# wildsonbbl/gnnepcsaft

Hardware: AMD Instinct MI355X
Metric: molecular graphs/sec (fwd+bwd) (higher is better)
Workload: dtype f32; 1 GPU; BASELINE configs[1]: PNA hidden=128 L=6 towers=1 pre=2 post=4, 4096 graphs/GPU (81920 atoms, 163840 directed bonds), fwd+loss+bwd incl. CSR packing; graphs_per_gpu=4096, parallelism=dp1, hip_graph=False, launch=auto, grad_allreduce_bytes=0, grad_exchange=none (1 rank)

## Files before the change

gnnepcsaft_amd/_lib.py:

```python
from __future__ import annotations

import ctypes as C
from pathlib import Path
from typing import Dict, Optional

import torch

_LIB_PATH = Path(__file__).resolve().parent / "libgnnepcsaft_hip.so"

ABI_VERSION = 7
GNX_OK, GNX_E_INVALID, GNX_E_HIP, GNX_E_RANGE, GNX_E_WORKSPACE = 0, -1, -2, -3, -4
OPT_GEMM_SPLIT, OPT_WGRAD_WGS, OPT_EMBED_BWD_MFMA, OPT_STD_BWD_CENTERED, OPT_GEMM_PIPE, OPT_WGRAD_PIPE, OPT_GEMM_AS, \
    OPT_GEMM_WS_FAST, OPT_GEMM_TILE_ROWS, OPT_GEMM_MID = range(10)
GEMM_RELU, GEMM_ACCUMULATE, GEMM_B_TRANS, GEMM_SPLIT_ONLY, GEMM_PRESPLIT = 1, 2, 4, 8, 16
GEMM_KERNEL_NAMES = ("none", "k_gemm<vec>", "k_gemm<generic>", "k_gemm_ws", "k_gemm_ws3", "k_gemm_ws3<fast,8>",
                     "k_gemm_ws3<fast,4>", "k_gemm3", "k_gemm3p<96>", "k_gemm3p<128>", "k_gemm_as3", "k_gemm_mid",
                     "k_gemm_small_batched")
POOL_ADD, POOL_MEAN, POOL_MAX = 0, 1, 2
K_NONE, K_PNA_AGG_FWD, K_PNA_AGG_BWD, K_GEMM_WS, K_GEMM_WGRAD, K_GINE_AGG_FWD, K_GINE_AGG_BWD, K_EDGE_COMBINE_FWD, \
    K_EDGE_COMBINE_BWD, K_BN_FWD, K_BN_BWD, K_GEMM_TILED, K_GEMM_SMALL, K_GEMM_WGRAD_BATCHED, K_KEY_SEGMENT_SUM, \
    K_EMBED, K_PNA_EDGE_FWD, K_PNA_EDGE_BWD, K_ATTN_FWD, K_ATTN_BWD, K_PCSAFT_RHO, K_PCSAFT_VP, \
    K_PCSAFT_MIX_STATE, K_PCSAFT_MIX_RHO, K_PCSAFT_MIX_LNPHI_STATE, K_PCSAFT_MIX_LNPHI = range(26)
K_COUNT = 26
KERNEL_GROUPS = {K_PNA_AGG_FWD: "pna_aggregate_fwd", K_PNA_AGG_BWD: "pna_aggregate_bwd", K_GEMM_WS: "gemm_weights_stationary",
                 K_GEMM_WGRAD: "weight_gradient", K_GINE_AGG_FWD: "gine_aggregate_fwd", K_GINE_AGG_BWD: "gine_aggregate_bwd",
                 K_EDGE_COMBINE_FWD: "edge_combine_fwd", K_EDGE_COMBINE_BWD: "edge_combine_bwd", K_BN_FWD: "batchnorm_fwd",
                 K_BN_BWD: "batchnorm_bwd", K_GEMM_TILED: "gemm_tiled", K_GEMM_SMALL: "gemm_small",
                 K_GEMM_WGRAD_BATCHED: "weight_gradient_batched", K_KEY_SEGMENT_SUM: "key_segment_sum", K_EMBED: "embedding",
                 K_PNA_EDGE_FWD: "pna_edge_fused_fwd", K_PNA_EDGE_BWD: "pna_edge_fused_bwd",
                 K_ATTN_FWD: "transformer_attn_fwd", K_ATTN_BWD: "transformer_attn_bwd",
                 K_PCSAFT_RHO: "pcsaft_density", K_PCSAFT_VP: "pcsaft_vapor_pressure",
                 K_PCSAFT_MIX_STATE: "pcsaft_mix_state", K_PCSAFT_MIX_RHO: "pcsaft_mix_density",
                 K_PCSAFT_MIX_LNPHI_STATE: "pcsaft_mix_lnphi_state", K_PCSAFT_MIX_LNPHI: "pcsaft_mix_lnphi"}


class GnxError(RuntimeError):
    def __init__(self, status: int, msg: str):
        super().__init__(f"gnx status {status}: {msg}")
        self.status = status


class GemmSeg(C.Structure):
    _fields_ = [("a", C.c_void_p), ("lda", C.c_int64), ("rowscale", C.c_void_p), ("b", C.c_void_p),
                ("ldb", C.c_int64), ("k", C.c_int32), ("_pad", C.c_int32)]


class GemmPlanInfo(C.Structure):
    _fields_ = [("kernel", C.c_int32), ("tile_rows", C.c_int32), ("grid_x", C.c_uint32), ("grid_y", C.c_uint32),
                ("block", C.c_uint32), ("runs_split", C.c_int32), ("image_bytes", C.c_size_t)]


class WgradProb(C.Structure):
    _fields_ = [("dC", C.c_void_p), ("lddc", C.c_int64), ("A", C.c_void_p), ("lda", C.c_int64),
                ("rowscale", C.c_void_p), ("dW", C.c_void_p), ("lddw", C.c_int64), ("dbias", C.c_void_p),
                ("M", C.c_int64), ("N", C.c_int32), ("K", C.c_int32)]


_vp, _i32, _i64, _f32, _sz = C.c_void_p, C.c_int32, C.c_int64, C.c_float, C.c_size_t

PNA_MAX_LAYERS, PNA_MAX_TOWERS = 8, 8
PNA_BWD_DEFER_SMALL, PNA_BWD_LAST_OF_PASS = 1, 2


class PnaFwdArgs(C.Structure):
    _fields_ = [("N", _i64), ("E", _i64), ("T", _i32), ("F", _i32), ("pre_layers", _i32), ("post_layers", _i32),
                ("D", _i32), ("merged", _i32),
                ("rowptr", _vp), ("src", _vp), ("dst", _vp), ("code", _vp), ("dperm", _vp), ("tiles", _vp), ("ntiles", _vp),
                ("max_tiles", _i64), ("x", _vp), ("Te", _vp), ("weff", _vp * PNA_MAX_TOWERS), ("Wm", _vp), ("bm", _vp),
                ("params", C.POINTER(_vp)), ("P", _vp), ("Q", _vp), ("A", _vp), ("hs", _vp * PNA_MAX_LAYERS),
                ("zs", _vp * PNA_MAX_LAYERS), ("ws", _vp), ("ws_bytes", _sz), ("out", _vp), ("etile_info", _vp),
                ("etile_w", _i32), ("tile_rows", _i32)]


class PnaBwdArgs(C.Structure):
    _fields_ = [("N", _i64), ("E", _i64), ("T", _i32), ("F", _i32), ("pre_layers", _i32), ("post_layers", _i32),
                ("R", _i32), ("D", _i32), ("avg_deg_log", _f32), ("merged", _i32), ("acc_first", _i32),
                ("use_side_streams", _i32), ("n_h", _i32), ("n_z", _i32),
                ("rowptr", _vp), ("colptr", _vp), ("cpos", _vp), ("code", _vp), ("code_pos", _vp), ("dperm", _vp),
                ("tiles", _vp), ("ntiles", _vp), ("chunks", _vp), ("nchunks", _vp),
                ("max_tiles", _i64), ("max_chunks", _i64),
                ("x", _vp), ("BE", _vp), ("EE", _vp), ("A", _vp),
                ("hs", _vp * PNA_MAX_LAYERS), ("zs", _vp * PNA_MAX_LAYERS), ("weff", _vp * PNA_MAX_TOWERS), ("Wm", _vp),
# ... 57 lines not shown
                             C.POINTER(C.c_double), C.POINTER(C.c_double)]),
    "gnx_prof_end": (_i32, [_vp]),
    "gnx_pack_csr_workspace_bytes": (_sz, [_i64, _i64]),
    "gnx_pack_csr": (_i32, [_vp, _vp, _i64, _i64, _vp, _vp, _vp, _vp, _vp, _vp, _vp, _sz]),
    "gnx_feature_code": (_i32, [_vp, _vp, _i64, _i32, C.POINTER(_i32), _vp, _vp, _vp, _sz]),
    "gnx_graph_ptr": (_i32, [_vp, _vp, _i64, _i64, _vp, _vp, _sz]),
    "gnx_degree_scalers": (_i32, [_vp, _vp, _i64, _f32, _vp, _vp]),
    "gnx_embed_sum_fwd": (_i32, [_vp, _vp, _i64, _i32, C.POINTER(_i32), _vp, _i32, _vp]),
    "gnx_table_scatter_workspace_bytes": (_sz, [_i64, _i32, _i32]),
    "gnx_embed_sum_bwd": (_i32, [_vp, _vp, _i64, _i32, C.POINTER(_i32), _i32, _vp, _i32, _vp, _vp, _sz]),
    "gnx_check_range": (_i32, [_vp]),
    "gnx_collate_ptr": (_i32, [_vp, _vp, _vp, _i64, _vp, _i64, _vp, _vp]),
    "gnx_collate_gather": (_i32, [_vp, _vp, _vp, _i64, _vp, _vp, _vp, _i64, _vp, _i64, _vp, _vp, _i64, _i64, _vp, _vp,
                                  _vp, _vp]),
    "gnx_collate_rows": (_i32, [_vp, _vp, _i64, _vp, _i64, _i32, _i32, _vp]),
    "gnx_gemm_workspace_bytes": (_sz, [_vp, _i32, C.POINTER(GemmSeg), C.POINTER(_i64), _i32, _i64, _i32, _vp, _i32,
                                       _i32]),
    "gnx_gemm": (_i32, [_vp, _i32, C.POINTER(GemmSeg), _i64, _i32, _vp, _vp, _i64, _vp, _i64, _i32, _vp, _sz]),
    "gnx_gemm_wgrad": (_i32, [_vp, _vp, _i64, _vp, _i64, _vp, _i64, _i32, _i32, _vp, _i64, _vp]),
    "gnx_gemm_wgrad_batched": (_i32, [_vp, _i32, C.POINTER(WgradProb)]),
    "gnx_degree_max": (_i32, [_vp, _vp, _i64, C.POINTER(_i32)]),
    "gnx_degree_classes_workspace_bytes": (_sz, [_i64, _i32]),
    "gnx_degree_classes": (_i32, [_vp, _vp, _i64, _i32, _vp, _vp, _vp, _sz]),
    "gnx_class_tiles": (_i32, [_vp, _vp, _i32, _i32, _vp, _vp]),
    "gnx_gemm_grouped": (_i32, [_vp, _i32, C.POINTER(GemmSeg), C.POINTER(_i64), _i32, _i64, _i32, _vp, _vp, _i64, _vp,
                                _i64, _i32, _vp, _vp, _vp, _i64, _vp, _sz]),
    "gnx_gemm_tile_rows": (_i32, [_vp, _i64, _i32]),
    "gnx_gemm_grouped_rows": (_i32, [_vp, _i32, C.POINTER(GemmSeg), C.POINTER(_i64), _i32, _i64, _i32, _vp, _vp, _i64, _vp,
                                     _i64, _i32, _vp, _vp, _vp, _i64, _vp, _sz, _i32]),
    "gnx_gemm_plan": (_i32, [_vp, _i32, C.POINTER(GemmSeg), C.POINTER(_i64), _i32, _i64, _i32, _vp, _vp, _i64, _vp, _i64, _i32,
                             _vp, _vp, _vp, _i64, _vp, _sz, _i32, C.POINTER(GemmPlanInfo)]),
    "gnx_gemm_wgrad_grouped": (_i32, [_vp, _vp, _i64, _vp, _i64, _i64, _i32, _i32, _vp, _i64, _i64, _vp, _vp, _vp,
                                      _i64]),
    "gnx_pna_weff": (_i32, [_vp, _vp, _i64, _i32, _i32, _f32, _vp]),
    "gnx_pna_weff_bwd": (_i32, [_vp, _vp, _i32, _i32, _f32, _vp, _i64]),
    "gnx_group_by_small_key": (_i32, [_vp, _vp, _i64, _i32, _vp, _vp, _vp, _sz]),
    "gnx_key_segment_sum": (_i32, [_vp, _vp, _vp, _vp, _i64, _i32, _vp]),
    "gnx_edge_combine_fwd": (_i32, [_vp, _vp, _vp, _vp, _vp, _vp, _vp, _i64, _i32, _i32, _vp]),
    "gnx_edge_combine_bwd": (_i32, [_vp, _vp, _vp, _vp, _vp, _vp, _i64, _i64, _i32, _i32, _vp, _vp, _vp, _vp, _sz]),
    "gnx_pna_aggregate_fwd": (_i32, [_vp, _vp, _vp, _i64, _i64, _i32, _i32, _vp]),
    "gnx_pna_aggregate_bwd": (_i32, [_vp, _vp, _vp, _vp, _vp, _i64, _i64, _i32, _i32, _vp]),
    "gnx_edge_tiles_count": (_i32, [_i64, _i32]),
    "gnx_edge_tiles": (_i32, [_vp, _vp, _i64, _i64, _i32, _vp]),
    "gnx_pack_batch_workspace_bytes": (_sz, [_i64, _i64, _i32, _i32]),
    "gnx_pack_batch": (_i32, [_vp, C.POINTER(PackBatchArgs)]),
    "gnx_pack_batch_scan_chunk": (_i64, []),
    "gnx_pack_batch_scan_bound": (_i64, []),
    "gnx_pna_edge_fwd": (_i32, [_vp, _vp, _vp, _vp, _vp, _vp, _vp, _vp, _vp, _i32, _i64, _i64, _i32, _i32, C.POINTER(_vp),
                                C.POINTER(_vp), _vp, _vp, _vp]),
    "gnx_pna_edge_bwd": (_i32, [_vp, _vp, _vp, _vp, _vp, _vp, _i32, _i64, _i64, _i32, _i32, _i32, C.POINTER(_vp), _vp, _vp,
                                _vp]),
    "gnx_gine_aggregate_fwd": (_i32, [_vp, _vp, _vp, _vp, _vp, _vp, _i64, _i64, _i32, _f32, _vp]),
    "gnx_gine_aggregate_bwd": (_i32, [_vp, _vp, _vp, _vp, _vp, _vp, _vp, _vp, _vp, _vp, _i64, _i64, _i32, _i32, _f32,
                                      _vp, _vp]),
    "gnx_gine_dle": (_i32, [_vp, _vp, _vp, _vp, _vp, _vp, _vp, _vp, _i64, _i32, _i32, _vp]),
    "gnx_transformer_attn_fwd": (_i32, [_vp, _vp, _vp, _vp, _vp, _vp, _i64, _i64, _i32, _i32, _f32, C.c_uint64,
                                        C.c_uint64, _vp, _vp, _vp]),
    "gnx_transformer_attn_bwd": (_i32, [_vp, _vp, _vp, _vp, _vp, _vp, _vp, _vp, _vp, _vp, _vp, _vp, _i64, _i64, _i32,
                                        _i32, _i32, _f32, C.c_uint64, C.c_uint64, _vp, _vp, _vp]),
    "gnx_transformer_attn_dle": (_i32, [_vp, _vp, _vp, _vp, _vp, _vp, _vp, _i64, _i32, _i32, _i32, _vp]),
    "gnx_pcsaft_density": (_i32, [_vp, _vp, _i64, _vp, _vp, _vp, _i64, _vp, _vp]),
    "gnx_pcsaft_vapor_pressure": (_i32, [_vp, _vp, _i64, _vp, _vp, _i64, _vp, _vp, _vp, _vp]),
    "gnx_pcsaft_mix_state": (_i32, [_vp, _vp, _i64, _vp, _vp, _vp, _i64, _i32, _vp, _vp, _vp, _vp, _i64, _vp, _vp, _vp,
                                    _vp]),
    "gnx_pcsaft_mix_density": (_i32, [_vp, _vp, _i64, _vp, _vp, _vp, _i64, _i32, _vp, _vp, _vp, _vp, _i64, _vp, _vp]),
    "gnx_pcsaft_mix_lnphi_state": (_i32, [_vp, _vp, _i64, _vp, _vp, _vp, _i64, _i32, _vp, _vp, _vp, _vp, _i64, _vp, _vp,
# ... 117 lines not shown
```

gnnepcsaft_amd/csrc/gnx_wgrad.hip:

```cpp
#include "gnx_split.hpp"

struct wgrad_args {
  const float* X;
  int64_t ldx;
  const float* Y;
  int64_t ldy;
  const float* rs;
  int64_t M;
  int N, K;
  float* dW;
  int64_t lddw;
  float* dbias;
  int64_t rows_per_block;
  int vec_x, vec_y;
  const int* row_index;
  const int* chunk_info;
  const int* nchunks;
  int64_t dw_cls_stride;
  const float* zero;
};

template <bool VEC, bool GROUPED>
__device__ __forceinline__ void wgrad_body(const wgrad_args& g, const int bx, const int by, const int bz, float* Xs,
                                           float* Ys) {
  const int tid = threadIdx.x;
  const int lane = tid & 63;
  const int wave = tid >> 6;
  const int wm = wave >> 1, wn = wave & 1;
  const int li = lane & 31, lh = lane >> 5;
  const int n0 = by * BN;
  const int c0 = bz * BN;
  if (n0 >= g.N || c0 >= g.K) return;
  int64_t r_begin = (int64_t)bx * g.rows_per_block;
// ... 285 lines not shown
      for (int mi = 0; mi < 2; ++mi)
#pragma unroll
        for (int ni = 0; ni < 2; ++ni) mfma_3x3(acc[mi][ni], a[mi], b[ni]);
    }
  }

#pragma unroll
  for (int mi = 0; mi < 2; ++mi)
#pragma unroll
    for (int ni = 0; ni < 2; ++ni) {
      int gc = c0 + wn * 64 + ni * 32 + li;
      if (gc >= g.K) continue;
#pragma unroll
      for (int r = 0; r < 16; ++r) {
        int gr = n0 + wm * 64 + mi * 32 + (r & 3) + 8 * (r >> 2) + 4 * lh;
        if (gr >= g.N) continue;
        atomicAdd(dW + (int64_t)gr * g.lddw + gc, acc[mi][ni][r]);
      }
    }
  if (g.dbias != nullptr && bz == 0 && x_ok) atomicAdd(g.dbias + n0 + col, bsum);
}

template <bool GROUPED>
__global__ void __launch_bounds__(256, 2) k_gemm_wgrad3(wgrad_args g) {
  __shared__ __attribute__((aligned(16))) unsigned char A3[G3_OP];
  __shared__ __attribute__((aligned(16))) unsigned char B3[G3_OP];
  __shared__ __attribute__((aligned(16))) unsigned offs[128];
  wgrad3_body<GROUPED>(g, blockIdx.x, blockIdx.y, blockIdx.z, A3, B3, offs);
}

#define WG3P_LDS (4 * G3_OP)
#define WG3P_NST 4

__device__ __forceinline__ void wgrad3p_body(const wgrad_args& g, const int bx, const int by, const int bz,
                                             unsigned char* lds) {
  const int tid = threadIdx.x;
  const int lane = tid & 63;
  const int wave = tid >> 6;
  const int n0 = by * BN;
  const int c0 = bz * BN;
  if (n0 >= g.N || c0 >= g.K) return;
  int64_t r_begin = (int64_t)bx * g.rows_per_block;
  int64_t r_end = r_begin + g.rows_per_block;
  if (r_end > g.M) r_end = g.M;
  float* const dW = g.dW;
  if (r_begin >= r_end) return;
  const int64_t nsteps = (r_end - r_begin + BK - 1) / BK;

  if (wave < 4) {
    const int wm = wave >> 1, wn = wave & 1;
    const int li = lane & 31, lh = lane >> 5;
    f32x16 acc[2][2];
#pragma unroll
    for (int i = 0; i < 2; ++i)
#pragma unroll
      for (int j = 0; j < 2; ++j)
#pragma unroll
        for (int r = 0; r < 16; ++r) acc[i][j][r] = 0.f;
    __syncthreads();
    for (int64_t j = 0; j < nsteps; ++j) {
      const unsigned char* const A3 = lds + (j & 1) * 2 * G3_OP;
      const unsigned char* const B3 = A3 + G3_OP;
#pragma unroll
      for (int sl = 0; sl < 2; ++sl) {
        bf16x8 a[2][3], b[2][3];
#pragma unroll
// ... 73 lines not shown
  load_step(std::integral_constant<int, 0>{}, row_of(0));
  load_step(std::integral_constant<int, 1>{}, row_of(1));
  load_step(std::integral_constant<int, 2>{}, row_of(2));
  load_step(std::integral_constant<int, 3>{}, row_of(3));
  store_step(std::integral_constant<int, 0>{}, lds);
  load_step(std::integral_constant<int, 0>{}, row_of(4));
  __syncthreads();

  auto iteration = [&](auto KC, int64_t j) {
    constexpr int K = decltype(KC)::value;
    constexpr int P = (K + 1) % WG3P_NST;
    store_step(std::integral_constant<int, P>{}, lds + ((K + 1) & 1) * 2 * G3_OP);
    load_step(std::integral_constant<int, P>{}, row_of(j + 1 + WG3P_NST));
    __syncthreads();
  };
  for (int64_t j = 0; j < nsteps; j += 4) {
    iteration(std::integral_constant<int, 0>{}, j);
    if (j + 1 >= nsteps) break;
    iteration(std::integral_constant<int, 1>{}, j + 1);
    if (j + 2 >= nsteps) break;
    iteration(std::integral_constant<int, 2>{}, j + 2);
    if (j + 3 >= nsteps) break;
    iteration(std::integral_constant<int, 3>{}, j + 3);
  }
  if (g.dbias != nullptr && bz == 0 && role == 0 && col_ok) {
#pragma unroll
    for (int q = 0; q < 4; ++q) atomicAdd(g.dbias + n0 + c4 + q, bsum[q]);
  }
}

__global__ void __launch_bounds__(512, 1) k_gemm_wgrad3p(wgrad_args g) {
  extern __shared__ __attribute__((aligned(16))) unsigned char lds_w[];
  wgrad3p_body(g, blockIdx.x, blockIdx.y, blockIdx.z, lds_w);
}

#define WGRAD_MAX_BATCH 8
struct wgrad_batch_args {
  wgrad_args p[WGRAD_MAX_BATCH];
  int nprob;
  int wg_off[WGRAD_MAX_BATCH + 1];
  int tiles_k[WGRAD_MAX_BATCH];
  int tiles[WGRAD_MAX_BATCH];
};

__device__ __forceinline__ void wgrad_batch_locate(const wgrad_batch_args& b, int w, int& prob, int& chunk, int& by,
                                                   int& bz) {
  prob = 0;
#pragma unroll
  for (int i = 1; i < WGRAD_MAX_BATCH; ++i) prob += (i < b.nprob && w >= b.wg_off[i]) ? 1 : 0;
  int off = b.wg_off[0], tiles = b.tiles[0], tk = b.tiles_k[0];
#pragma unroll
  for (int i = 1; i < WGRAD_MAX_BATCH; ++i)
    if (i == prob) {
      off = b.wg_off[i];
      tiles = b.tiles[i];
      tk = b.tiles_k[i];
    }
  const int local = w - off;
  chunk = local / tiles;
  const int t = local - chunk * tiles;
  by = t / tk;
  bz = t - by * tk;
}

__global__ void __launch_bounds__(256, 2) k_gemm_wgrad_batched(wgrad_batch_args b) {
  __shared__ __attribute__((aligned(16))) float Xs[BK * LDN];
// ... 20 lines not shown
}

__global__ void __launch_bounds__(512, 1) k_gemm_wgrad3p_batched(wgrad_batch_args b) {
  extern __shared__ __attribute__((aligned(16))) unsigned char lds_wb[];
  int prob, chunk, by, bz;
  wgrad_batch_locate(b, blockIdx.x, prob, chunk, by, bz);
  wgrad_args g = b.p[0];
#pragma unroll
  for (int i = 1; i < WGRAD_MAX_BATCH; ++i)
    if (i == prob) g = b.p[i];
  wgrad3p_body(g, chunk, by, bz, lds_wb);
}

static wgrad_args wgrad_args_of(const gnx_handle* h, const gnx_wgrad_prob& q) {
  wgrad_args g = {};
  g.X = q.dC;
  g.ldx = q.lddc;
  g.Y = q.A;
  g.ldy = q.lda;
  g.rs = q.rowscale;
  g.M = q.M;
  g.N = q.N;
  g.K = q.K;
  g.dW = q.dW;
  g.lddw = q.lddw;
  g.dbias = q.dbias;
  g.vec_x = aligned16(q.dC) && (q.lddc % 4 == 0);
  g.vec_y = aligned16(q.A) && (q.lda % 4 == 0);
  g.zero = h->d_zero;
  return g;
}

static bool wgrad_split_enabled(const gnx_handle* h, int64_t M, bool any_rowscale) {
  if (any_rowscale || M < 4096) return false;
  return h->opt[GNX_OPT_GEMM_SPLIT] != 0;
}

static int32_t wgrad_launch(gnx_handle* h, const float* dC, int64_t lddc, const float* A, int64_t lda,
                            const float* rowscale, int64_t M, int32_t N, int32_t K, float* dW, int64_t lddw,
                            float* dbias, const int32_t* row_index, const int32_t* chunk_info, const int32_t* nchunks,
                            int64_t max_chunks, int64_t dw_cls_stride) {
  GNX_CHECK_ARG(h && dC && A && dW, "gnx_gemm_wgrad: NULL argument");
  GNX_CHECK_ARG(M >= 0 && N > 0 && K > 0 && lddc >= N && lda >= K && lddw >= K, "gnx_gemm_wgrad: bad shape");
  if (M == 0) return GNX_OK;
  wgrad_args g = wgrad_args_of(h, gnx_wgrad_prob{dC, lddc, A, lda, rowscale, dW, lddw, dbias, M, N, K});
  int64_t tiles = gnx_cdiv(N, BN) * gnx_cdiv(K, BN);
  const int64_t target_wgs = h->opt[GNX_OPT_WGRAD_WGS] > 0 ? h->opt[GNX_OPT_WGRAD_WGS] : (h->num_cus > 0 ? h->num_cus : 256);
  int64_t chunks = gnx_cdiv(target_wgs, tiles);
  int64_t rows = gnx_cdiv(gnx_cdiv(M, chunks), BK) * BK;
  if (rows < 128) rows = 128;
  g.rows_per_block = rows;
  g.row_index = row_index;
  g.chunk_info = chunk_info;
  g.nchunks = nchunks;
  g.dw_cls_stride = dw_cls_stride;
  dim3 grid((unsigned)(chunk_info ? max_chunks : gnx_cdiv(M, rows)), (unsigned)gnx_cdiv(N, BN), (unsigned)gnx_cdiv(K, BN));
  const bool vec = g.vec_x && g.vec_y && (N % 4 == 0) && (K % 4 == 0);
  const bool offs32 = (uint64_t)M * (uint64_t)lddc < (1ull << 32) && (uint64_t)M * (uint64_t)lda < (1ull << 32);
  const bool wsplit = wgrad_split_enabled(h, M, rowscale != nullptr) && (!chunk_info || offs32);
  const double wfl = 2.0 * (double)M * N * K;
  gnx_prof_scope prof(h, GNX_K_GEMM_WGRAD, 4.0 * M * ((double)N + K) + 4.0 * N * K, wfl, wsplit ? 6.0 * wfl : 0.0);
  if (wsplit && vec && !chunk_info && rows >= 512 && h->opt[GNX_OPT_WGRAD_PIPE] != 0) {
    GNX_HIP(gnx_raise_lds_limit<&k_gemm_wgrad3p>((int)WG3P_LDS));
    hipLaunchKernelGGL(k_gemm_wgrad3p, grid, dim3(512), WG3P_LDS, h->stream, g);
  } else if (wsplit) {
    if (chunk_info)
      hipLaunchKernelGGL((k_gemm_wgrad3<true>), grid, dim3(256), 0, h->stream, g);
    else
      hipLaunchKernelGGL((k_gemm_wgrad3<false>), grid, dim3(256), 0, h->stream, g);
  } else if (chunk_info) {
    if (vec)
      hipLaunchKernelGGL((k_gemm_wgrad<true, true>), grid, dim3(256), 0, h->stream, g);
    else
      hipLaunchKernelGGL((k_gemm_wgrad<false, true>), grid, dim3(256), 0, h->stream, g);
  } else {
    if (vec)
      hipLaunchKernelGGL((k_gemm_wgrad<true, false>), grid, dim3(256), 0, h->stream, g);
    else
      hipLaunchKernelGGL((k_gemm_wgrad<false, false>), grid, dim3(256), 0, h->stream, g);
  }
  GNX_LAUNCH_CHECK();
  return GNX_OK;
}

extern "C" int32_t gnx_gemm_wgrad(gnx_handle* h, const float* dC, int64_t lddc, const float* A, int64_t lda,
                                  const float* rowscale, int64_t M, int32_t N, int32_t K, float* dW, int64_t lddw,
                                  float* dbias) {
  return wgrad_launch(h, dC, lddc, A, lda, rowscale, M, N, K, dW, lddw, dbias, nullptr, nullptr, nullptr, 0, 0);
}

extern "C" int32_t gnx_gemm_wgrad_grouped(gnx_handle* h, const float* dC, int64_t lddc, const float* A, int64_t lda,
                                          int64_t M, int32_t N, int32_t K, float* dW_cls, int64_t lddw,
                                          int64_t dw_cls_stride, const int32_t* row_index, const int32_t* chunk_info,
                                          const int32_t* nchunks, int64_t max_chunks) {
  GNX_CHECK_ARG(row_index && chunk_info && nchunks && max_chunks > 0, "gnx_gemm_wgrad_grouped: NULL argument");
  return wgrad_launch(h, dC, lddc, A, lda, nullptr, M, N, K, dW_cls, lddw, nullptr, row_index, chunk_info, nchunks,
                      max_chunks, dw_cls_stride);
}

extern "C" int32_t gnx_gemm_wgrad_batched(gnx_handle* h, int32_t nprob, const gnx_wgrad_prob* probs) {
  GNX_CHECK_ARG(h && probs && nprob >= 1 && nprob <= WGRAD_MAX_BATCH, "gnx_gemm_wgrad_batched: nprob must be in [1,%d]",
                WGRAD_MAX_BATCH);
  wgrad_batch_args b;
  int64_t maxM = 0;
  int maxN = 0, maxK = 0;
  for (int i = 0; i < nprob; ++i) {
    const gnx_wgrad_prob& q = probs[i];
    GNX_CHECK_ARG(q.dC && q.A && q.dW && q.M >= 0 && q.N > 0 && q.K > 0 && q.lddc >= q.N && q.lda >= q.K && q.lddw >= q.K,
                  "gnx_gemm_wgrad_batched: problem %d: bad argument", i);
    b.p[i] = wgrad_args_of(h, q);
    GNX_CHECK_ARG(b.p[i].vec_x && b.p[i].vec_y && (q.N % 4 == 0) && (q.K % 4 == 0),
                  "gnx_gemm_wgrad_batched: problem %d is not 16-byte aligned / multiple-of-4 shaped", i);
    if (q.M > maxM) maxM = q.M;
    if (q.N > maxN) maxN = q.N;
    if (q.K > maxK) maxK = q.K;
  }
  for (int i = nprob; i < WGRAD_MAX_BATCH; ++i) b.p[i] = b.p[0];
  if (maxM == 0) return GNX_OK;
  double total_cost = 0.0;
  for (int i = 0; i < nprob; ++i)
    total_cost += (double)b.p[i].M * (double)(gnx_cdiv(b.p[i].N, BN) * gnx_cdiv(b.p[i].K, BN));
  int off = 0;
  for (int i = 0; i < WGRAD_MAX_BATCH; ++i) {
    b.wg_off[i] = off;
    b.tiles[i] = 1;
    b.tiles_k[i] = 1;
    if (i >= nprob) continue;
    const int tn = (int)gnx_cdiv(b.p[i].N, BN), tk = (int)gnx_cdiv(b.p[i].K, BN);
    const int64_t M = b.p[i].M > 0 ? b.p[i].M : 1;
    const double cus_d = (double)(h->num_cus > 0 ? h->num_cus : 256);
// ... 37 lines not shown
```

gnnepcsaft_amd/ops.py:

```python
from __future__ import annotations

import ctypes as C
import threading
from typing import List, Optional, Sequence, Tuple

import torch

from . import _lib
from ._lib import GemmSeg, check, handle

_I32 = C.c_int32


def _f32(t: torch.Tensor, name: str) -> torch.Tensor:
    if t.dtype != torch.float32:
        raise _lib.GnxError(_lib.GNX_E_INVALID, f"{name}: expected float32, got {t.dtype}")
    return t


def _mat(t: torch.Tensor, name: str) -> Tuple[int, int]:
    if t.dtype is not torch.float32:
        raise _lib.GnxError(_lib.GNX_E_INVALID, f"{name}: expected float32, got {t.dtype}")
    shape, strides = t.shape, t.stride()
    if len(shape) != 2 or (shape[1] > 1 and strides[1] != 1):
# ... 447 lines not shown
                 mask: Optional[torch.Tensor] = None, relu: bool = False, b_trans: bool = True,
                 forward_tiles: bool = False) -> torch.Tensor:
    if out.size(0) == 0:
        return out
    a, _ws = _gemm_args(segs, out, dc, bias, mask, relu, False, b_trans, forward_tiles)
    lib = _lib.load()
    check(lib.gnx_gemm_grouped_rows(*a) if forward_tiles else lib.gnx_gemm_grouped(*a[:19]))
    return out


def gemm_plan(segs, out: torch.Tensor, *, bias: Optional[torch.Tensor] = None, mask: Optional[torch.Tensor] = None,
              relu: bool = False, accumulate: bool = False, b_trans: bool = True, dc: Optional[DegreeClasses] = None,
              forward_tiles: bool = False) -> Tuple[str, "_lib.GemmPlanInfo"]:
    a, _ws = _gemm_args(segs, out, dc, bias, mask, relu, accumulate, b_trans, forward_tiles)
    info = _lib.GemmPlanInfo()
    check(_lib.load().gnx_gemm_plan(*a, C.byref(info)))
    return _lib.GEMM_KERNEL_NAMES[info.kernel], info


def gemm_wgrad_grouped(dC: torch.Tensor, A: torch.Tensor, dW_cls: torch.Tensor, dc: DegreeClasses) -> None:
    M, N = dC.shape
    if M == 0:
        return
    xp, ldx = _mat(dC, "dC")
    ap, lda = _mat(A, "A")
    K = A.size(1)
    if dW_cls.shape != (dc.D, N, K) or not dW_cls.is_contiguous():
        raise _lib.GnxError(_lib.GNX_E_INVALID, f"dW_cls must be contiguous [{dc.D},{N},{K}], got {tuple(dW_cls.shape)}")
    check(_lib.load().gnx_gemm_wgrad_grouped(handle(dC.device), xp, ldx, ap, lda, M, N, K, dW_cls.data_ptr(), K, N * K,
                                             dc.dperm.data_ptr(), dc.chunks.data_ptr(), dc.nchunks.data_ptr(),
                                             dc.max_chunks))


def pna_weff(W: torch.Tensor, F: int, D: int, avg_deg_log: float) -> torch.Tensor:
    wp, ldw = _mat(W, "W")
    out = torch.empty(D, F, 4 * F, dtype=torch.float32, device=W.device)
    check(_lib.load().gnx_pna_weff(handle(W.device), wp, ldw, F, D, float(avg_deg_log), out.data_ptr()))
    return out


def pna_weff_bwd(dWeff: torch.Tensor, F: int, D: int, avg_deg_log: float, dW: torch.Tensor) -> None:
    wp, ldw = _mat(dW, "dW")
    check(_lib.load().gnx_pna_weff_bwd(handle(dW.device), dWeff.data_ptr(), F, D, float(avg_deg_log), wp, ldw))


_SIDE_ENABLED = False
_SIDE_PENDING = set()
_SIDE_KEEP: dict = {}


def set_wgrad_side_stream(enabled: bool) -> None:
    global _SIDE_ENABLED
    _SIDE_ENABLED = bool(enabled)


_JOIN_QUEUED = False


_SIDE_USED: dict = {}


def _join(idx: int, which: Optional[int] = None) -> None:
    dev = torch.device("cuda", idx)
    used = _SIDE_USED.get(idx, set())
    for w in sorted(used if which is None else (used & {which})):
        check(_lib.load().gnx_side_join_n(handle(dev), w))
# ... 721 lines not shown
```

include/gnx.h:

```cpp
#ifndef GNX_H_
#define GNX_H_

#include <stddef.h>
#include <stdint.h>

#ifdef __cplusplus
extern "C" {
#endif

#define GNX_ABI_VERSION 7

enum {
  GNX_OK = 0,
  GNX_E_INVALID = -1,
  GNX_E_HIP = -2,
  GNX_E_RANGE = -3,
  GNX_E_WORKSPACE = -4
};

typedef struct gnx_handle gnx_handle;

int32_t gnx_create(gnx_handle** out, int32_t device);
int32_t gnx_destroy(gnx_handle* h);
int32_t gnx_set_stream(gnx_handle* h, void* hip_stream);
// ... 147 lines not shown
                              size_t ws_bytes, int32_t tile_rows);
enum {
  GNX_GEMM_KERNEL_NONE = 0,
  GNX_GEMM_KERNEL_TILED_VEC = 1,
  GNX_GEMM_KERNEL_TILED_GENERIC = 2,
  GNX_GEMM_KERNEL_WS = 3,
  GNX_GEMM_KERNEL_WS3 = 4,
  GNX_GEMM_KERNEL_WS3_FAST8 = 5,
  GNX_GEMM_KERNEL_WS3_FAST4 = 6,
  GNX_GEMM_KERNEL_GEMM3 = 7,
  GNX_GEMM_KERNEL_GEMM3P_96 = 8,
  GNX_GEMM_KERNEL_GEMM3P_128 = 9,
  GNX_GEMM_KERNEL_AS3 = 10,
  GNX_GEMM_KERNEL_MID = 11,
  GNX_GEMM_KERNEL_SMALL = 12,
  GNX_GEMM_KERNEL_COUNT = 13
};
typedef struct {
  int32_t kernel;
  int32_t tile_rows;
  uint32_t grid_x, grid_y, block;
  int32_t runs_split;
  size_t image_bytes;
} gnx_gemm_plan_info;
int32_t gnx_gemm_plan(gnx_handle* h, int32_t nseg, const gnx_gemm_seg* segs, const int64_t* cls_strides,
                      int32_t num_classes, int64_t M, int32_t N, const float* bias, const float* mask, int64_t ldmask,
                      float* C, int64_t ldc, int32_t flags, const int32_t* row_index, const int32_t* tile_info,
                      const int32_t* ntiles, int64_t max_tiles, void* ws, size_t ws_bytes, int32_t tile_rows,
                      gnx_gemm_plan_info* out);
int32_t gnx_gemm_wgrad_grouped(gnx_handle* h, const float* dC, int64_t lddc, const float* A, int64_t lda, int64_t M,
                               int32_t N, int32_t K, float* dW_cls, int64_t lddw, int64_t dw_cls_stride,
                               const int32_t* row_index, const int32_t* chunk_info, const int32_t* nchunks,
                               int64_t max_chunks);
int32_t gnx_pna_weff(gnx_handle* h, const float* W, int64_t ldw, int32_t F, int32_t D, float avg_deg_log, float* Weff);
int32_t gnx_pna_weff_bwd(gnx_handle* h, const float* dWeff, int32_t F, int32_t D, float avg_deg_log, float* dW,
                         int64_t lddw);
int32_t gnx_pna_weff_batched(gnx_handle* h, int32_t n, const float* const* W, int64_t ldw, int32_t F, int32_t D,
                             const float* avg_deg_log, float* const* Weff);
int32_t gnx_pna_weff_bwd_batched(gnx_handle* h, int32_t n, const float* const* dWeff, int32_t F, int32_t D,
                                 const float* avg_deg_log, float* const* dW, int64_t lddw);

int32_t gnx_edge_combine_fwd(gnx_handle* h, const float* P, const float* Q, const float* Te, const int32_t* src,
                             const int32_t* dst, const int32_t* code, int64_t E, int32_t H, int32_t relu, float* h1);
int32_t gnx_edge_combine_bwd(gnx_handle* h, const float* g, const int32_t* rowptr, const int32_t* colptr,
                             const int32_t* cpos, const int32_t* code, int64_t N, int64_t E, int32_t H, int32_t R,
                             float* dP, float* dQ, float* dTe, void* ws, size_t ws_bytes);

int32_t gnx_group_by_small_key(gnx_handle* h, const int32_t* keys, int64_t E, int32_t R, int32_t* pos, int32_t* ptr,
                               void* ws, size_t ws_bytes);
int32_t gnx_key_segment_sum(gnx_handle* h, const float* g, const int32_t* pos, const int32_t* key, int64_t E, int32_t H,
                            float* dtable);

int32_t gnx_pna_aggregate_fwd(gnx_handle* h, const float* m, const int32_t* rowptr, int64_t N, int64_t E, int32_t T,
                              int32_t F, float* A);
int32_t gnx_pna_aggregate_bwd(gnx_handle* h, const float* dA, const float* m, const float* A, const int32_t* rowptr,
                              int64_t N, int64_t E, int32_t T, int32_t F, float* dm);

int32_t gnx_edge_tiles_count(int64_t E, int32_t tile_w);
int32_t gnx_edge_tiles(gnx_handle* h, const int32_t* rowptr, int64_t N, int64_t E, int32_t tile_w, int32_t* tile_info);

#define GNX_PACK_MAX_AVG 4
#define GNX_PACK_CLASSES 1u
#define GNX_PACK_CODE_INDEX 2u
#define GNX_PACK_EDGE_TILES 4u
#define GNX_PACK_TILED_SCAN 256u
typedef struct {
// ... 262 lines not shown
```

Baseline: 639,600 graphs/s.

## Add warp-specialized pipelined split-bf16 kernel for grouped weight gradients

```diff
diff --git a/gnnepcsaft_amd/_lib.py b/gnnepcsaft_amd/_lib.py
--- a/gnnepcsaft_amd/_lib.py
+++ b/gnnepcsaft_amd/_lib.py
@@ -16,6 +16,8 @@
 GEMM_KERNEL_NAMES = ("none", "k_gemm<vec>", "k_gemm<generic>", "k_gemm_ws", "k_gemm_ws3", "k_gemm_ws3<fast,8>",
                      "k_gemm_ws3<fast,4>", "k_gemm3", "k_gemm3p<96>", "k_gemm3p<128>", "k_gemm_as3", "k_gemm_mid",
                      "k_gemm_small_batched")
+WGRAD_KERNEL_NAMES = ("none", "k_gemm_wgrad<true,true>", "k_gemm_wgrad<false,true>", "k_gemm_wgrad3<true>",
+                      "k_gemm_wgrad3p_grouped")
 POOL_ADD, POOL_MEAN, POOL_MAX = 0, 1, 2
 K_NONE, K_PNA_AGG_FWD, K_PNA_AGG_BWD, K_GEMM_WS, K_GEMM_WGRAD, K_GINE_AGG_FWD, K_GINE_AGG_BWD, K_EDGE_COMBINE_FWD, \
     K_EDGE_COMBINE_BWD, K_BN_FWD, K_BN_BWD, K_GEMM_TILED, K_GEMM_SMALL, K_GEMM_WGRAD_BATCHED, K_KEY_SEGMENT_SUM, \
@@ -48,6 +50,11 @@
 class GemmPlanInfo(C.Structure):
     _fields_ = [("kernel", C.c_int32), ("tile_rows", C.c_int32), ("grid_x", C.c_uint32), ("grid_y", C.c_uint32),
                 ("block", C.c_uint32), ("runs_split", C.c_int32), ("image_bytes", C.c_size_t)]
+
+
+class WgradGroupedPlanInfo(C.Structure):
+    _fields_ = [("kernel", C.c_int32), ("ranges", C.c_int32), ("chunks_per_range", C.c_int32), ("grid_x", C.c_uint32),
+                ("grid_y", C.c_uint32), ("grid_z", C.c_uint32), ("block", C.c_uint32)]
 
 
 class WgradProb(C.Structure):
@@ -171,6 +178,8 @@
                              _vp, _vp, _vp, _i64, _vp, _sz, _i32, C.POINTER(GemmPlanInfo)]),
     "gnx_gemm_wgrad_grouped": (_i32, [_vp, _vp, _i64, _vp, _i64, _i64, _i32, _i32, _vp, _i64, _i64, _vp, _vp, _vp,
                                       _i64]),
+    "gnx_gemm_wgrad_grouped_plan": (_i32, [_vp, _i64, _i64, _vp, _vp, _i64, _i32, _i32, _i64,
+                                           C.POINTER(WgradGroupedPlanInfo)]),
     "gnx_pna_weff": (_i32, [_vp, _vp, _i64, _i32, _i32, _f32, _vp]),
     "gnx_pna_weff_bwd": (_i32, [_vp, _vp, _i32, _i32, _f32, _vp, _i64]),
     "gnx_group_by_small_key": (_i32, [_vp, _vp, _i64, _i32, _vp, _vp, _vp, _sz]),
diff --git a/gnnepcsaft_amd/csrc/gnx_wgrad.hip b/gnnepcsaft_amd/csrc/gnx_wgrad.hip
--- a/gnnepcsaft_amd/csrc/gnx_wgrad.hip
+++ b/gnnepcsaft_amd/csrc/gnx_wgrad.hip
@@ -1,4 +1,7 @@
 #include "gnx_split.hpp"
+#include "gnx_wgrad_plan.hpp"
+
+static_assert(WGRAD_PLAN_BN == BN, "gnx_wgrad_plan.hpp: dW tile");
 
 struct wgrad_args {
   const float* X;
@@ -350,6 +353,59 @@
 #define WG3P_LDS (4 * G3_OP)
 #define WG3P_NST 4
 
+__device__ __forceinline__ void wg3p_store_column(const float (&xa)[8], unsigned char* dst) {
+  bf16x8 p1, p2, p3;
+  split3(xa, p1, p2, p3);
+  *reinterpret_cast<bf16x8*>(dst) = p1;
+  *reinterpret_cast<bf16x8*>(dst + G3_PIECE) = p2;
+  *reinterpret_cast<bf16x8*>(dst + 2 * G3_PIECE) = p3;
+}
+
+__device__ __forceinline__ void wg3p_multiply_step(f32x16 (&acc)[2][2], const unsigned char* stage, const int wave,
+                                                   const int lane) {
+  const int wm = wave >> 1, wn = wave & 1;
+  const int li = lane & 31, lh = lane >> 5;
+  const unsigned char* const A3 = stage;
+  const unsigned char* const B3 = A3 + G3_OP;
+#pragma unroll
+  for (int sl = 0; sl < 2; ++sl) {
+    bf16x8 a[2][3], b[2][3];
+#pragma unroll
+    for (int mi = 0; mi < 2; ++mi)
+#pragma unroll
+      for (int p = 0; p < 3; ++p)
+        a[mi][p] = *reinterpret_cast<const bf16x8*>(A3 + p * G3_PIECE + (wm * 64 + mi * 32 + li) * G3_LDB + 32 * sl + 16 * lh);
+#pragma unroll
+    for (int ni = 0; ni < 2; ++ni)
+#pragma unroll
+      for (int p = 0; p < 3; ++p)
+        b[ni][p] = *reinterpret_cast<const bf16x8*>(B3 + p * G3_PIECE + (wn * 64 + ni * 32 + li) * G3_LDB + 32 * sl + 16 * lh);
+#pragma unroll
+    for (int mi = 0; mi < 2; ++mi)
+#pragma unroll
+      for (int ni = 0; ni < 2; ++ni) mfma_3x3(acc[mi][ni], a[mi], b[ni]);
+  }
+}
+
+__device__ __forceinline__ void wg3p_flush(const f32x16 (&acc)[2][2], const wgrad_args& g, float* dW, const int n0,
+                                           const int c0, const int wave, const int lane) {
+  const int wm = wave >> 1, wn = wave & 1;
+  const int li = lane & 31, lh = lane >> 5;
+#pragma unroll
+  for (int mi = 0; mi < 2; ++mi)
+#pragma unroll
+    for (int ni = 0; ni < 2; ++ni) {
+      int gc = c0 + wn * 64 + ni * 32 + li;
+      if (gc >= g.K) continue;
+#pragma unroll
+      for (int r = 0; r < 16; ++r) {
+        int gr = n0 + wm * 64 + mi * 32 + (r & 3) + 8 * (r >> 2) + 4 * lh;
+        if (gr >= g.N) continue;
+        atomicAdd(dW + (int64_t)gr * g.lddw + gc, acc[mi][ni][r]);
+      }
+    }
+}
+
 __device__ __forceinline__ void wgrad3p_body(const wgrad_args& g, const int bx, const int by, const int bz,
                                              unsigned char* lds) {
   const int tid = threadIdx.x;
@@ -489,6 +545,136 @@
 __global__ void __launch_bounds__(512, 1) k_gemm_wgrad3p(wgrad_args g) {
   extern __shared__ __attribute__((aligned(16))) unsigned char lds_w[];
   wgrad3p_body(g, blockIdx.x, blockIdx.y, blockIdx.z, lds_w);
+}
+
+#define WG3G_RING 16
+#define WG3G_LDS (WG3P_LDS + WG3G_RING * BK * 4)
+
+struct wgrad_grouped_args {
+  wgrad_args g;
+  int chunks_per_range;
+  int max_chunks;
+};
+
+__global__ void __launch_bounds__(512, 1) k_gemm_wgrad3p_grouped(wgrad_grouped_args ga) {
+  const wgrad_args& g = ga.g;
+  extern __shared__ __attribute__((aligned(16))) unsigned char lds_wg[];
+  unsigned char* const lds = lds_wg;
+  unsigned* const ring = reinterpret_cast<unsigned*>(lds_wg + WG3P_LDS);
+  const int tid = threadIdx.x;
+  const int lane = tid & 63;
+  const int wave = tid >> 6;
+  const int n0 = blockIdx.y * BN;
+  const int c0 = blockIdx.z * BN;
+  if (n0 >= g.N || c0 >= g.K) return;
+  const int c_begin = (int)blockIdx.x * ga.chunks_per_range;
+  int nch = __builtin_amdgcn_readfirstlane(g.nchunks[0]);
+  nch = nch < ga.max_chunks ? nch : ga.max_chunks;
+  const int c_end = c_begin + ga.chunks_per_range < nch ? c_begin + ga.chunks_per_range : nch;
+  auto info = [&](int i) { return __builtin_amdgcn_readfirstlane(g.chunk_info[i]); };
+  auto next_run = [&](int& c, int& p0, int& len, int& cls) {
+    p0 = info(3 * c);
+    len = info(3 * c + 1);
+    cls = info(3 * c + 2);
+    for (++c; c < c_end && info(3 * c + 2) == cls && info(3 * c) == p0 + len; ++c) len += info(3 * c + 1);
+  };
+  auto row_at = [&](int p0, int len, int i) { return (unsigned)g.row_index[p0 + (i < len ? i : 0)]; };
+
+  if (wave < 4) {
+    for (int c = c_begin; c < c_end;) {
+      int p0, len, cls;
+      next_run(c, p0, len, cls);
+      if (len <= 0) continue;
+      const int nsteps = (len + BK - 1) / BK;
+      f32x16 acc[2][2];
+#pragma unroll
+      for (int i = 0; i < 2; ++i)
+#pragma unroll
+        for (int j = 0; j < 2; ++j)
+#pragma unroll
+          for (int r = 0; r < 16; ++r) acc[i][j][r] = 0.f;
+      __syncthreads();
+      __syncthreads();
+      unsigned pend = 0;
+      for (int j = 0; j < nsteps; ++j) {
+        if ((j & 7) == 3) pend = row_at(p0, len, (j + 13) * BK + tid);
+        wg3p_multiply_step(acc, lds + (j & 1) * 2 * G3_OP, wave, lane);
+        if ((j & 7) == 4) ring[((j + 12) & (WG3G_RING - 1)) * BK + tid] = pend;
+        __syncthreads();
+      }
+      wg3p_flush(acc, g, g.dW + (int64_t)cls * g.dw_cls_stride, n0, c0, wave, lane);
+    }
+    return;
+  }
+
+  const int lt = tid - 256;
+  const int role = lt >> 7;
+  const int c4 = (lt & 31) * 4, rg = (lt >> 5) & 3;
+  const bool col_ok = role ? (c0 + c4 < g.K) : (n0 + c4 < g.N);
+  const float* const base = (role ? g.Y + (col_ok ? c0 + c4 : 0) : g.X + (col_ok ? n0 + c4 : 0));
+  const float* const zero = g.zero;
+  const unsigned ld = (unsigned)(role ? g.ldy : g.ldx);
+  const int img = role * G3_OP;
+  int len = 0;
+
+  f32x4 v[WG3P_NST][8];
+
+  auto load_step = [&](auto PC, int step) {
+    constexpr int P = decltype(PC)::value;
+    const int left = len - (step * BK + rg * 8);
+    const int nval = (left >= 8 && col_ok) ? 8 : ((left > 0 && col_ok) ? left : 0);
+    const unsigned* const rr = ring + (step & (WG3G_RING - 1)) * BK + rg * 8;
+    const split_u32x4 ra = *reinterpret_cast<const split_u32x4*>(rr);
+    const split_u32x4 rb = *reinterpret_cast<const split_u32x4*>(rr + 4);
+#pragma unroll
+    for (int j = 0; j < 8; ++j) {
+      const unsigned off = (j < 4 ? ra[j & 3] : rb[j & 3]) * ld;
+      v[P][j] = *reinterpret_cast<const f32x4*>(j < nval ? base + off : zero);
+    }
+  };
+  auto store_step = [&](auto PC, unsigned char* stage) {
+    constexpr int P = decltype(PC)::value;
+#pragma unroll
+    for (int q = 0; q < 4; ++q) {
+      float xa[8];
+#pragma unroll
+      for (int j = 0; j < 8; ++j) xa[j] = v[P][j][q];
+      wg3p_store_column(xa, stage + img + (c4 + q) * G3_LDB + rg * 16);
+    }
+  };
+  auto iteration = [&](auto KC, int j) {
+    constexpr int K = decltype(KC)::value;
+    constexpr int P = (K + 1) % WG3P_NST;
+    store_step(std::integral_constant<int, P>{}, lds + ((K + 1) & 1) * 2 * G3_OP);
+    load_step(std::integral_constant<int, P>{}, j + 1 + WG3P_NST);
+    __syncthreads();
+  };
+
+  for (int c = c_begin; c < c_end;) {
+    int p0, cls;
+    next_run(c, p0, len, cls);
+    if (len <= 0) continue;
+    const int nsteps = (len + BK - 1) / BK;
+    ring[lt] = row_at(p0, len, lt);
+    ring[256 + lt] = row_at(p0, len, 256 + lt);
+    __syncthreads();
+    load_step(std::integral_constant<int, 0>{}, 0);
+    load_step(std::integral_constant<int, 1>{}, 1);
+    load_step(std::integral_constant<int, 2>{}, 2);
+    load_step(std::integral_constant<int, 3>{}, 3);
+    store_step(std::integral_constant<int, 0>{}, lds);
+    load_step(std::integral_constant<int, 0>{}, 4);
+    __syncthreads();
+    for (int j = 0; j < nsteps; j += 4) {
+      iteration(std::integral_constant<int, 0>{}, j);
+      if (j + 1 >= nsteps) break;
+      iteration(std::integral_constant<int, 1>{}, j + 1);
+      if (j + 2 >= nsteps) break;
+      iteration(std::integral_constant<int, 2>{}, j + 2);
+      if (j + 3 >= nsteps) break;
+      iteration(std::integral_constant<int, 3>{}, j + 3);
+    }
+  }
 }
 
 #define WGRAD_MAX_BATCH 8
@@ -575,8 +761,7 @@
 }
 
 static bool wgrad_split_enabled(const gnx_handle* h, int64_t M, bool any_rowscale) {
-  if (any_rowscale || M < 4096) return false;
-  return h->opt[GNX_OPT_GEMM_SPLIT] != 0;
+  return wgrad_plan_split_enabled(h->opt, M, any_rowscale);
 }
 
 static int32_t wgrad_launch(gnx_handle* h, const float* dC, int64_t lddc, const float* A, int64_t lda,
@@ -603,7 +788,14 @@
   const bool wsplit = wgrad_split_enabled(h, M, rowscale != nullptr) && (!chunk_info || offs32);
   const double wfl = 2.0 * (double)M * N * K;
   gnx_prof_scope prof(h, GNX_K_GEMM_WGRAD, 4.0 * M * ((double)N + K) + 4.0 * N * K, wfl, wsplit ? 6.0 * wfl : 0.0);
-  if (wsplit && vec && !chunk_info && rows >= 512 && h->opt[GNX_OPT_WGRAD_PIPE] != 0) {
+  wgrad_grouped_plan p = {};
+  if (chunk_info) p = wgrad_grouped_plan_of(dC, lddc, A, lda, M, N, K, max_chunks, h->opt);
+  if (p.kernel == GNX_WGRAD_KERNEL_SPLIT3P_GROUPED) {
+    grid.x = p.grid_x;
+    GNX_HIP(gnx_raise_lds_limit<&k_gemm_wgrad3p_grouped>((int)WG3G_LDS));
+    hipLaunchKernelGGL(k_gemm_wgrad3p_grouped, grid, dim3(512), WG3G_LDS, h->stream,
+                       wgrad_grouped_args{g, p.chunks_per_range, (int)max_chunks});
+  } else if (wsplit && vec && !chunk_info && rows >= 512 && h->opt[GNX_OPT_WGRAD_PIPE] != 0) {
     GNX_HIP(gnx_raise_lds_limit<&k_gemm_wgrad3p>((int)WG3P_LDS));
     hipLaunchKernelGGL(k_gemm_wgrad3p, grid, dim3(512), WG3P_LDS, h->stream, g);
   } else if (wsplit) {
@@ -639,6 +831,23 @@
   GNX_CHECK_ARG(row_index && chunk_info && nchunks && max_chunks > 0, "gnx_gemm_wgrad_grouped: NULL argument");
   return wgrad_launch(h, dC, lddc, A, lda, nullptr, M, N, K, dW_cls, lddw, nullptr, row_index, chunk_info, nchunks,
                       max_chunks, dw_cls_stride);
+}
+
+extern "C" int32_t gnx_gemm_wgrad_grouped_plan(gnx_handle* h, int64_t lddc, int64_t lda, const float* dC, const float* A,
+                                               int64_t M, int32_t N, int32_t K, int64_t max_chunks,
+                                               gnx_wgrad_grouped_plan_info* out) {
+  GNX_CHECK_ARG(h && dC && A && out && max_chunks > 0, "gnx_gemm_wgrad_grouped_plan: NULL argument");
+  GNX_CHECK_ARG(M >= 0 && N > 0 && K > 0 && lddc >= N && lda >= K, "gnx_gemm_wgrad_grouped_plan: bad shape");
+  const wgrad_grouped_plan p = wgrad_grouped_plan_of(dC, lddc, A, lda, M, N, K, max_chunks, h->opt);
+  const bool pipe = p.kernel == GNX_WGRAD_KERNEL_SPLIT3P_GROUPED;
+  *out = gnx_wgrad_grouped_plan_info{p.kernel,
+                                     p.ranges,
+                                     p.chunks_per_range,
+                                     p.kernel == GNX_WGRAD_KERNEL_NONE ? 0u : p.grid_x,
+                                     (uint32_t)gnx_cdiv(N, BN),
+                                     (uint32_t)gnx_cdiv(K, BN),
+                                     pipe ? 512u : 256u};
+  return GNX_OK;
 }
 
 extern "C" int32_t gnx_gemm_wgrad_batched(gnx_handle* h, int32_t nprob, const gnx_wgrad_prob* probs) {
diff --git a/gnnepcsaft_amd/csrc/gnx_wgrad_plan.hpp b/gnnepcsaft_amd/csrc/gnx_wgrad_plan.hpp
--- /dev/null
+++ b/gnnepcsaft_amd/csrc/gnx_wgrad_plan.hpp
@@ -0,0 +1,48 @@
+#pragma once
+#include <cstdint>
+
+#include "gnx.h"
+
+constexpr int64_t WGRAD_PLAN_BN = 128;
+constexpr int64_t WGRAD_SPLIT_MIN_ROWS = 4096;
+constexpr int64_t WGRAD_GROUPED_WGS = 256;
+
+struct wgrad_grouped_plan {
+  int kernel = GNX_WGRAD_KERNEL_NONE;
+  int ranges = 1;
+  int chunks_per_range = 1;
+  unsigned grid_x = 0;
+};
+
+static inline int64_t wgrad_plan_cdiv(int64_t a, int64_t b) { return (a + b - 1) / b; }
+static inline bool wgrad_plan_vec(const void* p, int64_t ld) { return (reinterpret_cast<uintptr_t>(p) & 15) == 0 && ld % 4 == 0; }
+
+static inline bool wgrad_plan_split_enabled(const int* opt, int64_t M, bool any_rowscale) {
+  if (any_rowscale || M < WGRAD_SPLIT_MIN_ROWS) return false;
+  return opt[GNX_OPT_GEMM_SPLIT] != 0;
+}
+
+static inline wgrad_grouped_plan wgrad_grouped_plan_of(const float* dC, int64_t lddc, const float* A, int64_t lda, int64_t M,
+                                                       int32_t N, int32_t K, int64_t max_chunks, const int* opt) {
+  const bool vec = wgrad_plan_vec(dC, lddc) && wgrad_plan_vec(A, lda) && N % 4 == 0 && K % 4 == 0;
+  const bool offs32 = (uint64_t)M * (uint64_t)lddc < (1ull << 32) && (uint64_t)M * (uint64_t)lda < (1ull << 32);
+  const bool wsplit = wgrad_plan_split_enabled(opt, M, false) && offs32;
+  const int64_t tiles = wgrad_plan_cdiv(N, WGRAD_PLAN_BN) * wgrad_plan_cdiv(K, WGRAD_PLAN_BN);
+  const int64_t budget = opt[GNX_OPT_WGRAD_WGS] > 0 ? opt[GNX_OPT_WGRAD_WGS] : WGRAD_GROUPED_WGS;
+  wgrad_grouped_plan p;
+  p.ranges = (int)(budget / tiles > 1 ? budget / tiles : 1);
+  p.chunks_per_range = (int)wgrad_plan_cdiv(max_chunks, p.ranges);
+  if (M == 0)
+    p.kernel = GNX_WGRAD_KERNEL_NONE;
+  else if (wsplit && vec && opt[GNX_OPT_WGRAD_PIPE] != 0)
+    p.kernel = GNX_WGRAD_KERNEL_SPLIT3P_GROUPED;
+  else if (wsplit)
+    p.kernel = GNX_WGRAD_KERNEL_SPLIT3;
+  else
+    p.kernel = vec ? GNX_WGRAD_KERNEL_F32_VEC : GNX_WGRAD_KERNEL_F32_GENERIC;
+  if (p.kernel == GNX_WGRAD_KERNEL_SPLIT3P_GROUPED)
+    p.grid_x = (unsigned)wgrad_plan_cdiv(max_chunks, p.chunks_per_range);
+  else if (p.kernel != GNX_WGRAD_KERNEL_NONE)
+    p.grid_x = (unsigned)max_chunks;
+  return p;
+}
diff --git a/gnnepcsaft_amd/ops.py b/gnnepcsaft_amd/ops.py
--- a/gnnepcsaft_amd/ops.py
+++ b/gnnepcsaft_amd/ops.py
@@ -503,6 +503,15 @@
                                              dc.max_chunks))
 
 
+def gemm_wgrad_grouped_plan(dC: torch.Tensor, A: torch.Tensor, max_chunks: int) -> Tuple[str, "_lib.WgradGroupedPlanInfo"]:
+    xp, ldx = _mat(dC, "dC")
+    ap, lda = _mat(A, "A")
+    info = _lib.WgradGroupedPlanInfo()
+    check(_lib.load().gnx_gemm_wgrad_grouped_plan(handle(dC.device), ldx, lda, xp, ap, dC.size(0), dC.size(1), A.size(1),
+                                                  int(max_chunks), C.byref(info)))
+    return _lib.WGRAD_KERNEL_NAMES[info.kernel], info
+
+
 def pna_weff(W: torch.Tensor, F: int, D: int, avg_deg_log: float) -> torch.Tensor:
     wp, ldw = _mat(W, "W")
     out = torch.empty(D, F, 4 * F, dtype=torch.float32, device=W.device)
diff --git a/include/gnx.h b/include/gnx.h
--- a/include/gnx.h
+++ b/include/gnx.h
@@ -203,6 +203,21 @@
                                int32_t N, int32_t K, float* dW_cls, int64_t lddw, int64_t dw_cls_stride,
                                const int32_t* row_index, const int32_t* chunk_info, const int32_t* nchunks,
                                int64_t max_chunks);
+enum {
+  GNX_WGRAD_KERNEL_NONE = 0,
+  GNX_WGRAD_KERNEL_F32_VEC = 1,
+  GNX_WGRAD_KERNEL_F32_GENERIC = 2,
+  GNX_WGRAD_KERNEL_SPLIT3 = 3,
+  GNX_WGRAD_KERNEL_SPLIT3P_GROUPED = 4,
+  GNX_WGRAD_KERNEL_COUNT = 5
+};
+typedef struct {
+  int32_t kernel;
+  int32_t ranges, chunks_per_range;
+  uint32_t grid_x, grid_y, grid_z, block;
+} gnx_wgrad_grouped_plan_info;
+int32_t gnx_gemm_wgrad_grouped_plan(gnx_handle* h, int64_t lddc, int64_t lda, const float* dC, const float* A, int64_t M,
+                                    int32_t N, int32_t K, int64_t max_chunks, gnx_wgrad_grouped_plan_info* out);
 int32_t gnx_pna_weff(gnx_handle* h, const float* W, int64_t ldw, int32_t F, int32_t D, float avg_deg_log, float* Weff);
 int32_t gnx_pna_weff_bwd(gnx_handle* h, const float* dWeff, int32_t F, int32_t D, float avg_deg_log, float* dW,
                          int64_t lddw);
```

Result: faster. 647,900 graphs/s, median of 6 (+1.3%).
